# BlueAnon/BD-BNN

Measured on AMD Instinct MI355X. Metric: train_images_per_sec, higher is better.
Workload: dtype bf16; 1 GPU; model=resnet18_bdbnn, global_batch=2048, image=3x224x224, kurtosis=True, parallelism=dp1

## Files before the change

bdbnn_amd/csrc/api.h:

```cpp
#pragma once
#include <hip/hip_runtime.h>
#include <cstdint>

constexpr int BDBNN_MAX_TENSORS = 64;

struct TensorListArg {
  const float* ptr[BDBNN_MAX_TENSORS];
  int64_t numel[BDBNN_MAX_TENSORS];
  int n;
};

struct PtrList { float* ptr[BDBNN_MAX_TENSORS]; };

constexpr int64_t BDBNN_CHUNK_ELEMS = 32 * 1024;

constexpr int bdbnn_bn_sum_rows(int act_kind) {
  return act_kind == 3 ? 4 : 3;
}

extern "C" {

void bdbnn_sign_pack(const void* x, uint32_t* out, int64_t pixels, int C,
                     int CW, bool bf16, hipStream_t stream);
void bdbnn_binsign_decode(const void* x, void* y, int64_t n, bool in_bf16,
                          bool out_bf16, hipStream_t stream);
void bdbnn_ste_mask_mul(const void* g, const void* x, void* y, int64_t n,
                        bool g_bf16, bool x_bf16, int mode, float t, float k,
                        hipStream_t stream);
void bdbnn_weight_pack(const float* w, uint32_t* wp, float* alpha,
                       float* stab, int K, int C, int KH, int KW, int CW,
                       hipStream_t stream);
void bdbnn_sign_mask_pack(const void* x, uint32_t* sp, uint32_t* mp,
                          int64_t pixels, int C, int CW, bool bf16,
                          hipStream_t stream);
void bdbnn_decode_packed(const uint32_t* sp, void* y, int64_t pixels, int C,
                         int CW, bool out_bf16, hipStream_t stream);
void bdbnn_mask_mul_packed(const void* g, const uint32_t* mp, void* dx,
                           int64_t pixels, int C, int CW, bool g_bf16,
                           bool out_bf16, hipStream_t stream);
void bdbnn_weight_decode(const uint32_t* wp, const float* alpha, void* w,
                         int K, int C, int T, int CW, bool out_bf16,
                         hipStream_t stream);

void bdbnn_xnor_conv_fwd(
    const uint32_t* xp, const uint32_t* wp, const float* alpha,
    const float* stab, void* out, float* s1, float* s2, bool out_bf16,
    int N, int H, int W, int C, int K, int KH, int KW, int stride, int pad,
    int Ho, int Wo, hipStream_t stream);

void bdbnn_stem_pack_x4(const void* x, void* x4, int64_t npix, bool bf16,
                        hipStream_t stream);
void bdbnn_stem_pack_w4(const float* w, void* w4T, hipStream_t stream);
void bdbnn_stem_fwd(const void* x4, const void* w4T, void* out, int N, int H,
                    int W, hipStream_t stream);
int bdbnn_stem_wrw_nslab(int N, int H, int W);
void bdbnn_stem_wrw(const void* x4, const void* g, float* dwslab, int N,
                    int H, int W, hipStream_t stream);
void bdbnn_stem_fold_dw4(const float* slabs, float* dw, int nslab,
                         hipStream_t stream);

void bdbnn_kd_logit_fwd(const void* s, const void* t, float* stats,
                        float* out, int B, int C, bool bf16,
                        hipStream_t stream);
void bdbnn_kd_logit_bwd(const void* s, const void* t, const float* stats,
                        void* ds, float gscale, int B, int C, bool bf16,
                        hipStream_t stream);
void bdbnn_ce_fwd(const void* s, const int64_t* y, float* stats, float* out,
                  int B, int C, bool bf16, hipStream_t stream);
void bdbnn_ce_bwd(const void* s, const int64_t* y, const float* stats,
                  void* ds, float gscale, int B, int C, bool bf16,
                  hipStream_t stream);

void bdbnn_maxpool_fwd(const void* x, void* out, unsigned char* idx, int N,
                       int C, int H, int W, int Ho, int Wo, int ks,
                       int stride, int pad, bool bf16, hipStream_t stream);
void bdbnn_maxpool_bwd(const void* dy, const unsigned char* idx, void* dx,
                       int N, int C, int H, int W, int Ho, int Wo, int ks,
                       int stride, int pad, bool bf16, hipStream_t stream);

void bdbnn_prelu_fwd(const void* x, const float* a, void* y, int64_t n,
                     int C, bool bf16, hipStream_t stream);
void bdbnn_prelu_bwd(const void* x, const void* g, const float* a, void* dx,
                     float* da, int64_t n, int C, bool bf16,
                     hipStream_t stream);

void bdbnn_bn_stats(const void* x, float* s1, float* s2, int64_t n, int C,
                    bool bf16, hipStream_t stream);
void bdbnn_bn_finalize(const float* s1, const float* s2, float* mean,
                       float* invstd, float* running_mean,
                       float* running_var, int C, float n, float momentum,
                       float eps, int nslice, hipStream_t stream);
void bdbnn_bn_act_fwd(const void* x, const void* skip, const float* mean,
                      const float* invstd, const float* gamma,
                      const float* beta, const float* a, const float* b1,
                      const float* b2, void* out, void* zout, int64_t n,
                      int C, int act_kind, uint32_t* xpk, uint32_t* mpk,
                      bool bf16, hipStream_t stream);
void bdbnn_bn_act_bwd_reduce(const void* dy, const void* z, const void* x,
                             const float* mean, const float* invstd,
                             const float* a, float* sums32, float* sums,
                             int64_t n, int C, int act_kind, bool bf16,
                             hipStream_t stream);
void bdbnn_bn_fold_sums(const float* sums32, float* sums, int n,
                        hipStream_t stream);
void bdbnn_bn_act_bwd_apply(const void* dy, const void* z, const void* x,
                            const float* mean, const float* invstd,
                            const float* gamma, const float* a,
                            const float* sums, void* dx, void* dskip,
                            int64_t n, int C, int act_kind, float inv_n,
                            bool bf16, hipStream_t stream);
void bdbnn_bn_act_eval(const void* x, const void* skip, const float* rm,
                       const float* rv, const float* gamma,
                       const float* beta, const float* a, const float* b1,
                       const float* b2, void* out, int64_t n, int C,
                       int act_kind, float eps, bool bf16,
                       hipStream_t stream);

void bdbnn_bn_relu_maxpool_fwd(
    const void* x, const float* mean, const float* invstd,
    const float* gamma, const float* beta, void* out, unsigned char* idx,
    uint32_t* xpk, uint32_t* mpk, int N, int C, int H, int W, int Ho, int Wo,
    int ks, int stride, int pad, bool bf16, hipStream_t stream);
void bdbnn_bn_relu_maxpool_bwd_reduce(
    const void* dy, const unsigned char* idx, const void* x,
    const float* mean, const float* invstd, const float* gamma,
    const float* beta, float* sums32, float* sums, int N, int C, int H,
    int W, int Ho, int Wo, int ks, int stride, int pad, bool bf16,
    hipStream_t stream);
void bdbnn_bn_relu_maxpool_bwd_apply(
    const void* dy, const unsigned char* idx, const void* x,
    const float* mean, const float* invstd, const float* gamma,
// ... 61 lines not shown
```

bdbnn_amd/csrc/bind.cpp:

```cpp
#include <torch/extension.h>
#include <c10/hip/HIPStream.h>
#include <hip/hip_runtime.h>

#include <string>
#include <unordered_map>
#include <utility>
#include <vector>

#include "api.h"

namespace {

hipStream_t cur_stream() {
  return c10::hip::getCurrentHIPStream().stream();
}

bool is_bf16(const at::Tensor& t) { return t.scalar_type() == at::kBFloat16; }

void check_vec8(const at::Tensor& t, bool vec8_c, const char* name,
                const char* who) {
  TORCH_CHECK(t.is_cuda() && (t.scalar_type() == at::kBFloat16 ||
                              t.scalar_type() == at::kFloat),
              who, ": ", name, " must be a bf16 or fp32 CUDA tensor");
  if (vec8_c) {
    TORCH_CHECK(t.dim() == 4, who, ": ", name, " must be 4-D (N,C,H,W)");
    int64_t C = t.size(1);
    TORCH_CHECK(C >= 8 && C <= 1024 && (C & (C - 1)) == 0, who,
                ": C must be a power of two, 8 <= C <= 1024");
  }
}

struct Schedule {
  at::Tensor bt, bo;
  int n_blocks;
};

Schedule build_schedule_uncached(const std::vector<at::Tensor>& ts,
                                 int64_t chunk_elems, const at::Device& dev) {
  std::vector<int> bt;
  std::vector<int64_t> bo;
  for (size_t l = 0; l < ts.size(); ++l) {
    int64_t n = ts[l].numel();
    for (int64_t off = 0; off < n; off += chunk_elems) {
      bt.push_back((int)l);
      bo.push_back(off);
    }
  }
  Schedule s;
  s.n_blocks = (int)bt.size();
  s.bt = at::from_blob(bt.data(), {(int64_t)bt.size()},
                       at::TensorOptions().dtype(at::kInt))
             .to(dev, false);
  s.bo = at::from_blob(bo.data(), {(int64_t)bo.size()},
                       at::TensorOptions().dtype(at::kLong))
             .to(dev, false);
  return s;
}

Schedule build_schedule(const std::vector<at::Tensor>& ts,
                        int64_t chunk_elems, const at::Device& dev) {
  static std::unordered_map<std::string, Schedule> cache;
  std::string key;
  key.reserve(ts.size() * 9 + 16);
  key += std::to_string(chunk_elems);
  key += '/';
  key += std::to_string(dev.index());
  for (auto& t : ts) {
    key += ':';
    key += std::to_string(t.numel());
  }
  auto it = cache.find(key);
  if (it != cache.end()) return it->second;
  if (cache.size() > 256) cache.clear();
  auto s = build_schedule_uncached(ts, chunk_elems, dev);
  cache.emplace(std::move(key), s);
  return s;
}

TensorListArg make_meta(const std::vector<at::Tensor>& ts) {
  TORCH_CHECK((int)ts.size() <= BDBNN_MAX_TENSORS,
              "too many tensors for one fused call");
  TensorListArg a;
  a.n = (int)ts.size();
  for (size_t i = 0; i < ts.size(); ++i) {
    TORCH_CHECK((ts[i].is_contiguous() ||
                 ts[i].is_contiguous(at::MemoryFormat::ChannelsLast)) &&
// ... 159 lines not shown

at::Tensor ste_mask_mul(const at::Tensor& g, const at::Tensor& x, int mode,
                        double t, double k) {
  TORCH_CHECK(g.is_cuda() && x.is_cuda() && g.numel() == x.numel(),
              "ste_mask_mul: matching CUDA tensors");
  check_vec8(g, false, "g", "ste_mask_mul");
  check_vec8(x, false, "x", "ste_mask_mul");
  TORCH_CHECK(x.numel() % 8 == 0, "ste_mask_mul: numel % 8 == 0");
  auto fmt = x.dim() == 4 ? at::MemoryFormat::ChannelsLast
                          : at::MemoryFormat::Contiguous;
  auto xc = x.contiguous(fmt);
  auto gc = g.contiguous(fmt);
  auto out = at::empty_like(xc, xc.options(), fmt);
  bdbnn_ste_mask_mul(gc.data_ptr(), xc.data_ptr(), out.data_ptr(),
                     xc.numel(), is_bf16(gc), is_bf16(xc), mode, (float)t,
                     (float)k, cur_stream());
  return out;
}


std::vector<at::Tensor> sign_mask_pack_nhwc(const at::Tensor& x) {
  TORCH_CHECK(x.is_cuda() && x.dim() == 4, "sign_mask_pack: 4-D CUDA tensor");
  check_vec8(x, false, "x", "sign_mask_pack");
  TORCH_CHECK(x.is_contiguous(at::MemoryFormat::ChannelsLast),
              "sign_mask_pack: channels_last input required");
  int64_t N = x.size(0), C = x.size(1), H = x.size(2), W = x.size(3);
  int CW = (int)((C + 31) / 32);
  auto sp = at::empty({N, H, W, CW}, x.options().dtype(at::kInt));
  auto mp = at::empty({N, H, W, CW}, x.options().dtype(at::kInt));
  bdbnn_sign_mask_pack(x.data_ptr(), (uint32_t*)sp.data_ptr<int>(),
                       (uint32_t*)mp.data_ptr<int>(), N * H * W, (int)C, CW,
                       is_bf16(x), cur_stream());
  return {sp, mp};
}

at::Tensor decode_packed(const at::Tensor& sp, int64_t C, bool out_bf16) {
  TORCH_CHECK(sp.is_cuda() && sp.dim() == 4 && sp.scalar_type() == at::kInt,
              "decode_packed: int32 [N,H,W,CW]");
  int64_t N = sp.size(0), H = sp.size(1), W = sp.size(2);
  int CW = (int)sp.size(3);
  auto out = at::empty({N, C, H, W},
                       sp.options().dtype(out_bf16 ? at::kBFloat16
                                                   : at::kFloat),
                       at::MemoryFormat::ChannelsLast);
  bdbnn_decode_packed((const uint32_t*)sp.data_ptr<int>(), out.data_ptr(),
                      N * H * W, (int)C, CW, out_bf16, cur_stream());
  return out;
}

at::Tensor mask_mul_packed(const at::Tensor& g, const at::Tensor& mp,
                           int64_t C, bool out_bf16) {
  TORCH_CHECK(g.is_cuda() && mp.is_cuda(), "mask_mul_packed: CUDA tensors");
  check_vec8(g, false, "g", "mask_mul_packed");
  auto gc = g.contiguous(at::MemoryFormat::ChannelsLast);
  int64_t N = mp.size(0), H = mp.size(1), W = mp.size(2);
  int CW = (int)mp.size(3);
  TORCH_CHECK(gc.numel() == N * H * W * C, "mask_mul_packed: shape mismatch");
  auto out = at::empty({N, C, H, W},
                       g.options().dtype(out_bf16 ? at::kBFloat16
                                                  : at::kFloat),
                       at::MemoryFormat::ChannelsLast);
  bdbnn_mask_mul_packed(gc.data_ptr(), (const uint32_t*)mp.data_ptr<int>(),
                        out.data_ptr(), N * H * W, (int)C, CW, is_bf16(gc),
                        out_bf16, cur_stream());
  return out;
}

at::Tensor weight_decode(const at::Tensor& wp, const at::Tensor& alpha,
                         int64_t C, bool out_bf16) {
  TORCH_CHECK(wp.is_cuda() && wp.dim() == 4 && wp.scalar_type() == at::kInt,
              "weight_decode: int32 [K,KH,KW,CW]");
  int K = (int)wp.size(0), KH = (int)wp.size(1), KW = (int)wp.size(2);
  int CW = (int)wp.size(3);
  auto out = at::empty({K, C, KH, KW},
                       wp.options().dtype(out_bf16 ? at::kBFloat16
                                                   : at::kFloat));
  bdbnn_weight_decode((const uint32_t*)wp.data_ptr<int>(),
                      alpha.data_ptr<float>(), out.data_ptr(), K, (int)C,
                      KH * KW, CW, out_bf16, cur_stream());
  return out;
}


std::vector<at::Tensor> xnor_conv_fwd(
    const at::Tensor& xp, const at::Tensor& wp, const at::Tensor& alpha,
    const at::Tensor& stab, int64_t C, int64_t stride, int64_t pad,
    bool out_bf16, bool want_stats) {
  TORCH_CHECK(xp.is_cuda() && xp.dim() == 4 && xp.scalar_type() == at::kInt,
              "xnor_conv: packed activations int32 [N,H,W,CW]");
  TORCH_CHECK(wp.dim() == 4, "xnor_conv: packed weights [K,KH,KW,CW]");
  int N = (int)xp.size(0), H = (int)xp.size(1), W = (int)xp.size(2);
  int K = (int)wp.size(0), KH = (int)wp.size(1), KW = (int)wp.size(2);
  TORCH_CHECK(KH * KW * wp.size(3) <= 160,
              "xnor_conv: KH*KW*ceil(C/32) must be <= 160 "
              "(kernel address-table size; C <= 512 at 3x3)");
  int Ho = (int)((H + 2 * pad - KH) / stride + 1);
  int Wo = (int)((W + 2 * pad - KW) / stride + 1);
  auto out = at::empty({N, K, Ho, Wo},
                       xp.options().dtype(out_bf16 ? at::kBFloat16
                                                   : at::kFloat),
                       at::MemoryFormat::ChannelsLast);
  at::Tensor s1, s2;
  float *s1p = nullptr, *s2p = nullptr;
  if (want_stats) {
    auto fopt = xp.options().dtype(at::kFloat);
    s1 = at::empty({32, K}, fopt);
    s2 = at::empty({32, K}, fopt);
    s1p = s1.data_ptr<float>();
    s2p = s2.data_ptr<float>();
  }
  bdbnn_xnor_conv_fwd((const uint32_t*)xp.data_ptr<int>(),
                      (const uint32_t*)wp.data_ptr<int>(),
                      alpha.data_ptr<float>(), stab.data_ptr<float>(),
                      out.data_ptr(), s1p, s2p, out_bf16, N, H, W, (int)C,
                      K, KH, KW, (int)stride, (int)pad, Ho, Wo,
                      cur_stream());
  if (want_stats) return {out, s1, s2};
  return {out};
}



std::vector<at::Tensor> stem_conv_fwd(const at::Tensor& x,
                                      const at::Tensor& w) {
  TORCH_CHECK(x.is_cuda() && x.dim() == 4 && x.size(1) == 3,
              "stem: (N,3,H,W) input");
  TORCH_CHECK(w.dim() == 4 && w.size(0) == 64 && w.size(1) == 3 &&
                  w.size(2) == 7 && w.size(3) == 7,
              "stem: (64,3,7,7) weights");
  int N = (int)x.size(0), H = (int)x.size(2), W = (int)x.size(3);
  TORCH_CHECK(H % 2 == 0 && W % 2 == 0, "stem: even H,W");
  auto xc = x.contiguous(at::MemoryFormat::ChannelsLast);
  bool bf16 = is_bf16(xc);
  auto bopt = xc.options().dtype(at::kBFloat16);
  auto x4 = at::empty({N, H, W, 4}, bopt);
  bdbnn_stem_pack_x4(xc.data_ptr(), x4.data_ptr(), (int64_t)N * H * W,
                     bf16, cur_stream());
  auto wf = w.contiguous().to(at::kFloat);
  auto w4T = at::empty({64, 224}, bopt);
  bdbnn_stem_pack_w4(wf.data_ptr<float>(), w4T.data_ptr(), cur_stream());
  auto out = at::empty({N, 64, H / 2, W / 2}, bopt,
                       at::MemoryFormat::ChannelsLast);
  bdbnn_stem_fwd(x4.data_ptr(), w4T.data_ptr(), out.data_ptr(), N, H, W,
                 cur_stream());
  return {out, x4};
}

at::Tensor stem_conv_wrw(const at::Tensor& x4, const at::Tensor& gy) {
  TORCH_CHECK(x4.is_cuda() && x4.dim() == 4 && x4.size(3) == 4 &&
                  x4.scalar_type() == at::kBFloat16,
              "stem wrw: packed x4 (N,H,W,4) bf16");
  int N = (int)x4.size(0), H = (int)x4.size(1), W = (int)x4.size(2);
  auto gc = gy.to(at::kBFloat16).contiguous(at::MemoryFormat::ChannelsLast);
  TORCH_CHECK(gc.size(1) == 64 && gc.size(2) == H / 2 &&
                  gc.size(3) == W / 2, "stem wrw: grad shape");
  int nslab = bdbnn_stem_wrw_nslab(N, H, W);
  auto fopt = x4.options().dtype(at::kFloat);
  auto slabs = at::empty({nslab, 64, 224}, fopt);
  bdbnn_stem_wrw(x4.data_ptr(), gc.data_ptr(), slabs.data_ptr<float>(),
                 N, H, W, cur_stream());
  auto dw = at::empty({64, 3, 7, 7}, fopt);
  bdbnn_stem_fold_dw4(slabs.data_ptr<float>(), dw.data_ptr<float>(),
                      nslab, cur_stream());
  return dw;
}


std::vector<at::Tensor> kd_logit_fwd(const at::Tensor& s,
                                     const at::Tensor& t) {
  check_logits(s, "kd_logit_fwd");
  TORCH_CHECK(t.is_cuda() && s.sizes() == t.sizes(),
              "kd_logit_fwd: teacher logits must be a CUDA tensor of the "
              "student's shape");
  auto sc = s.contiguous();
  auto tc = t.to(s.scalar_type()).contiguous();
  int B = (int)s.size(0), C = (int)s.size(1);
  auto fopt = sc.options().dtype(at::kFloat);
  auto stats = at::empty({B, 4}, fopt);
  auto out = at::empty({}, fopt);
  bdbnn_kd_logit_fwd(sc.data_ptr(), tc.data_ptr(), stats.data_ptr<float>(),
                     out.data_ptr<float>(), B, C, is_bf16(sc),
                     cur_stream());
  return {out, stats, tc};
}

at::Tensor kd_logit_bwd(const at::Tensor& s, const at::Tensor& t,
                        const at::Tensor& stats, double gscale) {
  check_logits(s, "kd_logit_bwd");
  TORCH_CHECK(t.is_cuda() && t.scalar_type() == s.scalar_type() &&
                  t.sizes() == s.sizes() && t.is_contiguous(),
              "kd_logit_bwd: t must be contiguous, of s's dtype and shape");
  TORCH_CHECK(stats.is_cuda() && stats.scalar_type() == at::kFloat &&
                  stats.is_contiguous() && stats.numel() == 4 * s.size(0),
              "kd_logit_bwd: stats must be contiguous fp32 [B,4]");
  auto sc = s.contiguous();
  int B = (int)s.size(0), C = (int)s.size(1);
  auto ds = at::empty_like(sc);
  bdbnn_kd_logit_bwd(sc.data_ptr(), t.data_ptr(), stats.data_ptr<float>(),
                     ds.data_ptr(), (float)(gscale / B), B, C, is_bf16(sc),
                     cur_stream());
  return ds;
// ... 738 lines not shown
  auto st = stats.contiguous();
  auto gs = gscale.to(dev, at::kFloat).contiguous();
  bdbnn_kurtosis_bwd(&meta, &gp, sched.bt.data_ptr<int>(),
                     sched.bo.data_ptr<int64_t>(), sched.n_blocks,
                     st.data_ptr<float>(), tgt.data_ptr<float>(),
                     gs.data_ptr<float>(), cur_stream());
  return grads;
}


at::Tensor weight_kd_fwd(const std::vector<at::Tensor>& ws,
                         const std::vector<at::Tensor>& wt) {
  auto meta = make_meta(ws);
  auto sched = build_schedule(ws, BDBNN_CHUNK_ELEMS, ws[0].device());
  auto s_ptr = make_ptrs(ws, meta, ws);
  auto t_ptr = make_ptrs(wt, meta, ws);
  auto out = at::zeros({}, ws[0].options().dtype(at::kDouble));
  bdbnn_weight_kd_fwd(&meta, &s_ptr, &t_ptr, sched.bt.data_ptr<int>(),
                      sched.bo.data_ptr<int64_t>(), sched.n_blocks,
                      out.data_ptr<double>(), cur_stream());
  return out.to(at::kFloat);
}

std::vector<at::Tensor> weight_kd_bwd(const std::vector<at::Tensor>& wt,
                                      const at::Tensor& gscale) {
  auto meta = make_meta(wt);
  auto sched = build_schedule(wt, BDBNN_CHUNK_ELEMS, wt[0].device());
  auto t_ptr = make_ptrs(wt, meta, wt);
  std::vector<at::Tensor> grads;
  for (auto& t : wt)
    grads.push_back(at::empty_like(t, t.options(),
                                   at::MemoryFormat::Preserve));
  auto gp = make_ptrs(grads, meta, wt);
  auto gs = gscale.to(wt[0].device(), at::kFloat).contiguous();
  bdbnn_weight_kd_bwd(&meta, &t_ptr, &gp, sched.bt.data_ptr<int>(),
                      sched.bo.data_ptr<int64_t>(), sched.n_blocks,
                      gs.data_ptr<float>(), cur_stream());
  return grads;
}


void fused_sgd(const std::vector<at::Tensor>& p,
               const std::vector<at::Tensor>& g,
               const std::vector<at::Tensor>& buf, double lr, double momentum,
               double wd) {
  auto meta = make_meta(p);
  auto sched = build_schedule(p, BDBNN_CHUNK_ELEMS, p[0].device());
  auto pp = make_ptrs(p, meta, p);
  auto gg = make_ptrs(g, meta, p);
  auto bb = make_ptrs(buf, meta, p);
  bdbnn_fused_sgd(&meta, &pp, &gg, &bb, sched.bt.data_ptr<int>(),
                  sched.bo.data_ptr<int64_t>(), sched.n_blocks, (float)lr,
                  (float)momentum, (float)wd, cur_stream());
}

void fused_adam(const std::vector<at::Tensor>& p,
                const std::vector<at::Tensor>& g,
                const std::vector<at::Tensor>& m1,
                const std::vector<at::Tensor>& m2, double lr, double beta1,
                double beta2, double eps, double wd, double bc1, double bc2) {
  auto meta = make_meta(p);
  auto sched = build_schedule(p, BDBNN_CHUNK_ELEMS, p[0].device());
  auto pp = make_ptrs(p, meta, p);
  auto gg = make_ptrs(g, meta, p);
  auto mm1 = make_ptrs(m1, meta, p);
  auto mm2 = make_ptrs(m2, meta, p);
  bdbnn_fused_adam(&meta, &pp, &gg, &mm1, &mm2, sched.bt.data_ptr<int>(),
                   sched.bo.data_ptr<int64_t>(), sched.n_blocks, (float)lr,
                   (float)beta1, (float)beta2, (float)eps, (float)wd,
                   (float)bc1, (float)bc2, cur_stream());
}

PYBIND11_MODULE(TORCH_EXTENSION_NAME, m) {
  m.def("sign_pack_nhwc", &sign_pack_nhwc, "sign+bitpack NHWC activations");
  m.def("weight_pack", &weight_pack,
        "pack conv weights -> (bits, alpha, pad-correction table)");
  m.def("binsign_decode", &binsign_decode, "elementwise +-1 decode");
  m.def("ste_mask_mul", &ste_mask_mul, "quantizer backward mask multiply");
  m.def("sign_mask_pack_nhwc", &sign_mask_pack_nhwc,
        "pack sign + clip-STE mask bitplanes in one pass");
  m.def("decode_packed", &decode_packed, "packed signs -> +-1 NHWC tensor");
  m.def("mask_mul_packed", &mask_mul_packed, "dx = mask_bit ? g : 0");
  m.def("weight_decode", &weight_decode, "packed weights -> alpha*(+-1)");
  m.def("xnor_conv_fwd", &xnor_conv_fwd, "bit-packed XNOR+popcount conv");
  m.def("stem_conv_fwd", &stem_conv_fwd,
        "MFMA 7x7/2 stem conv fwd (returns out, packed x4)");
  m.def("stem_conv_wrw", &stem_conv_wrw, "MFMA stem conv weight grad");
  m.def("kd_logit_fwd", &kd_logit_fwd, "fused logit-KD fwd");
  m.def("kd_logit_bwd", &kd_logit_bwd, "fused logit-KD bwd");
  m.def("ce_fwd", &ce_fwd, "fused cross-entropy fwd");
  m.def("ce_bwd", &ce_bwd, "fused cross-entropy bwd");
  m.def("maxpool_fwd", &maxpool_fwd, "fused NHWC maxpool fwd (+u8 idx)");
  m.def("maxpool_bwd", &maxpool_bwd, "gather-based NHWC maxpool bwd");
  m.def("prelu_fwd", &prelu_fwd, "fused NHWC per-channel PReLU fwd");
  m.def("prelu_bwd", &prelu_bwd, "fused NHWC per-channel PReLU bwd");
  m.def("bn_act_fwd_train", &bn_act_fwd_train,
        "fused BN(+add)(+act) training forward -> [out, z, mean, invstd(, "
        "xpk, mpk)]; act_kind 3 (RPReLU) takes b1, b2 and stores u = z + b1 "
        "as z",
        py::arg("x"), py::arg("skip"), py::arg("gamma"), py::arg("beta"),
        py::arg("a"), py::arg("running_mean"), py::arg("running_var"),
        py::arg("momentum"), py::arg("eps"), py::arg("act_kind"),
        py::arg("pre_s1"), py::arg("pre_s2"), py::arg("want_pack"),
        py::arg("b1") = py::none(), py::arg("b2") = py::none());
  m.def("bn_act_bwd", &bn_act_bwd,
        "fused BN(+add)(+act) backward -> [dx, dskip, dgamma, dbeta, da]; "
        "act_kind 3 appends db1, db2");
  m.def("bn_act_eval", &bn_act_eval, "fused BN(+add)(+act) eval forward",
        py::arg("x"), py::arg("skip"), py::arg("gamma"), py::arg("beta"),
        py::arg("a"), py::arg("rm"), py::arg("rv"), py::arg("eps"),
        py::arg("act_kind"), py::arg("b1") = py::none(),
        py::arg("b2") = py::none());
  m.def("bn_relu_maxpool_fwd_train", &bn_relu_maxpool_fwd_train,
        "fused BN + ReLU + maxpool training forward -> [out, idx, mean, "
        "invstd(, xpk, mpk)]",
        py::arg("x"), py::arg("gamma"), py::arg("beta"),
        py::arg("running_mean"), py::arg("running_var"),
        py::arg("momentum"), py::arg("eps"), py::arg("ks"),
        py::arg("stride"), py::arg("pad"), py::arg("pre_s1") = py::none(),
        py::arg("pre_s2") = py::none(), py::arg("want_pack") = false);
  m.def("bn_relu_maxpool_bwd", &bn_relu_maxpool_bwd,
        "fused BN + ReLU + maxpool backward -> [dx, dgamma, dbeta]");
  m.def("conv_dgrad2", &conv_dgrad2,
        "MFMA bf16 dgrad v2: halo-staged 9-tap implicit GEMM with fused "
        "clip-STE mask (3x3/s1/p1); optional acc adds a same-shape "
        "skip-gradient tensor in the epilogue",
        py::arg("g"), py::arg("wd"), py::arg("mp"), py::arg("C"),
        py::arg("acc") = py::none());
  m.def("conv_dgrad2_x", &conv_dgrad2_x,
        "conv_dgrad2 with a value mask of the saved bf16 activation x in "
        "the epilogue: mode 1 = ReAct polynomial, 2 = EDE(t, k)",
        py::arg("g"), py::arg("wd"), py::arg("x"), py::arg("C"),
        py::arg("mode"), py::arg("t"), py::arg("k"),
        py::arg("acc") = py::none());
  m.def("dgrad_weight_decode", &dgrad_weight_decode,
        "packed bits -> mirrored transposed +-alpha bf16 [9][C][K]");
  m.def("dgrad2_supported",
        [](int64_t H, int64_t W, int64_t C, int64_t K) {
          return bdbnn_dgrad2_supported((int)H, (int)W, (int)C, (int)K) !=
                 0;
        },
        "shape support predicate for conv_dgrad2");
  m.def("conv_wgrad2", &conv_wgrad2,
        "MFMA bf16 wgrad v2: all-9-tap block GEMM from sign BITS "
        "(3x3/s1/p1) -> fp32 [9][C][K]");
  m.def("repack_cplane", &repack_cplane,
        "activation sign bits -> padded per-channel u64 row planes");
  m.def("wgrad_finish", &wgrad_finish,
        "dwT transpose to [K][C][3][3] + |w|<=1 STE mask, one pass");
  m.def("dgrad2_s2_supported",
        [](int64_t H, int64_t W, int64_t C, int64_t K, int64_t ks) {
          return dgrad2_s2_routed(H, W, C, K, ks);
        },
        "routing predicate of the stride-2 MFMA backward; H, W are the "
        "input (dx) size, ks in {3 (pad 1), 1 (pad 0)}; false also for "
        "the shapes the kernels run but lose on (3x3 with C >= 128 and "
        "K >= 256)",
        py::arg("H"), py::arg("W"), py::arg("C"), py::arg("K"),
        py::arg("ks"));
  m.def("conv_dgrad2_s2", &conv_dgrad2_s2,
        "MFMA bf16 dgrad of a 3x3/s2/p1 (wd [9][C][K]) or 1x1/s2/p0 (wd "
        "[1][C][K]) binary conv by pixel parity; mode 0 masks with the "
        "bitplane mp, modes 1/2 with the value mask of x; optional acc "
        "adds a same-shape skip-gradient tensor in the epilogue",
        py::arg("g"), py::arg("wd"), py::arg("H"), py::arg("W"),
        py::arg("C"), py::arg("mode"), py::arg("mp"), py::arg("x"),
        py::arg("t"), py::arg("k"), py::arg("acc") = py::none());
// ... 21 lines not shown
```

bdbnn_amd/csrc/xnor_conv.hip:

```cpp
#include "common.h"
#include <cstdlib>

#define TILE_K 64
#define CHUNK 8
#define W_PER_THREAD 2
#define MAX_WORDS 160

struct XnorConvParams {
  int N, H, W, C, K, KH, KW, stride, pad, Ho, Wo, CW;
  int WORDS;
  int T;
  int base;
};

template <typename TO, bool STATS, int TM>
__global__ __launch_bounds__(256) void xnor_conv_kernel(
    const uint32_t* __restrict__ xp, const uint32_t* __restrict__ wp,
    const float* __restrict__ alpha, const float* __restrict__ stab,
    TO* __restrict__ out, float* __restrict__ s1, float* __restrict__ s2,
    XnorConvParams p, int grid_m) {
  const int wg = bd_xcd_remap(blockIdx.x, gridDim.x);
  int m_blk = wg % grid_m;
  int k_blk = wg / grid_m;
  const int tid = threadIdx.x;
  const int64_t M = (int64_t)p.N * p.Ho * p.Wo;
  const int64_t m0 = (int64_t)m_blk * TM;
  const int k0_blk = k_blk * TILE_K;

  constexpr int APT = CHUNK * TM / 256;
  constexpr int RPT = TM / 16;
  __shared__ uint32_t a_lds[2][CHUNK][TM];
  __shared__ uint32_t w_lds[2][CHUNK][TILE_K];
  __shared__ int row_basecw[TM];
  __shared__ unsigned short row_inv[TM];
  __shared__ int off_tab[MAX_WORDS];
  __shared__ unsigned char tap_tab[MAX_WORDS];
  __shared__ float csum[2][TILE_K];

  for (int r = tid; r < TM; r += blockDim.x) {
    int64_t sp = m0 + r;
    if (sp >= M) { row_basecw[r] = 0; row_inv[r] = 0xffff; continue; }
    int n = int(sp / ((int64_t)p.Ho * p.Wo));
    int rem = int(sp % ((int64_t)p.Ho * p.Wo));
    int oy = rem / p.Wo, ox = rem % p.Wo;
    int iy0 = oy * p.stride - p.pad;
    int ix0 = ox * p.stride - p.pad;
    row_basecw[r] = ((n * p.H + iy0) * p.W + ix0) * p.CW;
    unsigned short inv = 0;
    for (int t = 0; t < p.T; ++t) {
      int kh = t / p.KW, kw = t % p.KW;
      int iy = iy0 + kh, ix = ix0 + kw;
      if (iy < 0 || iy >= p.H || ix < 0 || ix >= p.W) inv |= 1u << t;
    }
    row_inv[r] = inv;
  }
  for (int wdx = tid; wdx < p.WORDS; wdx += blockDim.x) {
    int t = wdx / p.CW, cw = wdx - t * p.CW;
    int kh = t / p.KW, kw = t - kh * p.KW;
    off_tab[wdx] = (kh * p.W + kw) * p.CW + cw;
    tap_tab[wdx] = (unsigned char)t;
  }
  if constexpr (STATS)
    for (int c = tid; c < TILE_K; c += blockDim.x) {
      csum[0][c] = 0.f; csum[1][c] = 0.f;
    }
  __syncthreads();

  const int r0 = (tid / 16) * RPT;
  const int kq = (tid % 16) * 4;
  int acc[RPT][4] = {};

  int a_c[APT], a_r[APT];
#pragma unroll
  for (int it = 0; it < APT; ++it) {
    int j = tid + it * 256;
    a_c[it] = j / TM;
    a_r[it] = j % TM;
  }
  int w_c[W_PER_THREAD], w_k[W_PER_THREAD];
#pragma unroll
  for (int it = 0; it < W_PER_THREAD; ++it) {
    int j = tid + it * 256;
    w_c[it] = j / TILE_K;
    w_k[it] = j % TILE_K;
  }

  const int n_chunks = (p.WORDS + CHUNK - 1) / CHUNK;
  uint32_t av[APT], wv[W_PER_THREAD];

#define STAGE_LOAD(w0)                                                    \
  {                                                                       \
    _Pragma("unroll")                                                     \
    for (int it = 0; it < APT; ++it) {                                    \
      int widx = (w0) + a_c[it];                                          \
      int r = a_r[it];                                                    \
      uint32_t v = 0;                                                     \
      if (widx < p.WORDS && !((row_inv[r] >> tap_tab[widx]) & 1))         \
        v = xp[(int64_t)row_basecw[r] + off_tab[widx]];                   \
      av[it] = v;                                                         \
    }                                                                     \
    _Pragma("unroll")                                                     \
    for (int it = 0; it < W_PER_THREAD; ++it) {                           \
      int widx = (w0) + w_c[it];                                          \
      int kg = k0_blk + w_k[it];                                          \
      uint32_t v = 0;                                                     \
      if (widx < p.WORDS && kg < p.K)                                     \
        v = wp[(int64_t)kg * p.WORDS + widx];                             \
      wv[it] = v;                                                         \
    }                                                                     \
  }

#define STAGE_WRITE(buf)                                                  \
  {                                                                       \
    _Pragma("unroll")                                                     \
    for (int it = 0; it < APT; ++it)                                      \
      a_lds[buf][a_c[it]][a_r[it]] = av[it];                              \
    _Pragma("unroll")                                                     \
    for (int it = 0; it < W_PER_THREAD; ++it)                             \
      w_lds[buf][w_c[it]][w_k[it]] = wv[it];                              \
  }

  STAGE_LOAD(0);
  STAGE_WRITE(0);
  __syncthreads();

  for (int ch = 0; ch < n_chunks; ++ch) {
    const int buf = ch & 1;
    const bool more = ch + 1 < n_chunks;
    if (more) STAGE_LOAD((ch + 1) * CHUNK);
#pragma unroll
    for (int c = 0; c < CHUNK; ++c) {
// ... 137 lines not shown
```

setup.py:

```python

import os

from setuptools import setup

os.environ.setdefault("PYTORCH_ROCM_ARCH", "gfx950")

from torch.utils.cpp_extension import BuildExtension, CUDAExtension

ROOT = os.path.dirname(os.path.abspath(__file__))
CSRC = os.path.join(ROOT, "bdbnn_amd", "csrc")

sources = [os.path.join(CSRC, f) for f in (
    "bind.cpp",
    "pack.hip",
    "prelu.hip",
    "bn_act.hip",
    "bn_pool.hip",
    "pool.hip",
    "loss.hip",
    "conv_bwd.hip",
    "conv_bwd_s2.hip",
    "stem_conv.hip",
    "xnor_conv.hip",
    "kurtosis.hip",
    "kd.hip",
    "optim.hip",
)]

setup(
    name="bdbnn_amd_native",
    ext_modules=[
        CUDAExtension(
            name="bdbnn_amd._native",
            sources=sources,
            extra_compile_args={
                "cxx": ["-O3", "-std=c++17"],
                "nvcc": ["-O3", "-std=c++17"],
            },
        )
    ],
    cmdclass={"build_ext": BuildExtension.with_options(no_python_abi_suffix=False)},
)
```

Before: 25150 images/s.

## Add i8 MFMA binary conv forward kernel routed for 3x3 shapes

Adds a new forward kernel for binary 3x3 convolutions (stride 1 or 2, pad 1). It expands bit-packed signs into ±1 int8 in LDS, using halo tiles with swizzled slots, and accumulates with 32x32x32 i8 MFMA instructions instead of XNOR+popcount on the vector ALUs. The bind layer sends calls to it automatically when no BN statistics are requested and the channel counts are multiples of 64; an env var can turn this off, and the old kernel's invalid-tap mask is widened to 32 bits. The trade is an 8x expansion of the operand bytes written to LDS, plus a path that only runs when the stats epilogue is not needed.

```diff
diff --git a/bdbnn_amd/csrc/api.h b/bdbnn_amd/csrc/api.h
--- a/bdbnn_amd/csrc/api.h
+++ b/bdbnn_amd/csrc/api.h
@@ -47,6 +47,15 @@
     const float* stab, void* out, float* s1, float* s2, bool out_bf16,
     int N, int H, int W, int C, int K, int KH, int KW, int stride, int pad,
     int Ho, int Wo, hipStream_t stream);
+
+int bdbnn_xnor_mfma_supported(int C, int K, int KH, int KW, int stride,
+                              int pad);
+int bdbnn_xnor_mfma_routed(int C, int K, int KH, int KW, int stride,
+                           int pad);
+int bdbnn_xnor_conv_mfma_fwd(
+    const uint32_t* xp, const uint32_t* wp, const float* alpha, void* out,
+    bool out_bf16, int N, int H, int W, int C, int K, int KH, int KW,
+    int stride, int pad, int Ho, int Wo, hipStream_t stream);
 
 void bdbnn_stem_pack_x4(const void* x, void* x4, int64_t npix, bool bf16,
                         hipStream_t stream);
diff --git a/bdbnn_amd/csrc/bind.cpp b/bdbnn_amd/csrc/bind.cpp
--- a/bdbnn_amd/csrc/bind.cpp
+++ b/bdbnn_amd/csrc/bind.cpp
@@ -2,6 +2,7 @@
 #include <c10/hip/HIPStream.h>
 #include <hip/hip_runtime.h>
 
+#include <atomic>
 #include <string>
 #include <unordered_map>
 #include <utility>
@@ -327,10 +328,14 @@
 }
 
 
-std::vector<at::Tensor> xnor_conv_fwd(
+enum XnorRoute { kAuto, kMfma, kValu };
+
+static std::atomic<int64_t> g_xnor_route_calls[2];
+
+std::vector<at::Tensor> xnor_conv_route(
     const at::Tensor& xp, const at::Tensor& wp, const at::Tensor& alpha,
     const at::Tensor& stab, int64_t C, int64_t stride, int64_t pad,
-    bool out_bf16, bool want_stats) {
+    bool out_bf16, bool want_stats, XnorRoute route) {
   TORCH_CHECK(xp.is_cuda() && xp.dim() == 4 && xp.scalar_type() == at::kInt,
               "xnor_conv: packed activations int32 [N,H,W,CW]");
   TORCH_CHECK(wp.dim() == 4, "xnor_conv: packed weights [K,KH,KW,CW]");
@@ -339,6 +344,8 @@
   TORCH_CHECK(KH * KW * wp.size(3) <= 160,
               "xnor_conv: KH*KW*ceil(C/32) must be <= 160 "
               "(kernel address-table size; C <= 512 at 3x3)");
+  TORCH_CHECK(KH * KW <= 32,
+              "xnor_conv: at most 32 taps (invalid-tap bitmask width)");
   int Ho = (int)((H + 2 * pad - KH) / stride + 1);
   int Wo = (int)((W + 2 * pad - KW) / stride + 1);
   auto out = at::empty({N, K, Ho, Wo},
@@ -354,14 +361,71 @@
     s1p = s1.data_ptr<float>();
     s2p = s2.data_ptr<float>();
   }
+  bool mfma = route == kMfma;
+  if (route == kAuto)
+    mfma = !want_stats && bdbnn_xnor_mfma_routed((int)C, K, KH, KW,
+                                                 (int)stride, (int)pad);
+  if (mfma) {
+    TORCH_CHECK(!want_stats, "xnor_conv_mfma: no BN statistics epilogue");
+    TORCH_CHECK(wp.size(3) * 32 == C && xp.size(3) == wp.size(3),
+                "xnor_conv_mfma: C must equal 32 * CW of both operands");
+    int rc = bdbnn_xnor_conv_mfma_fwd(
+        (const uint32_t*)xp.data_ptr<int>(),
+        (const uint32_t*)wp.data_ptr<int>(), alpha.data_ptr<float>(),
+        out.data_ptr(), out_bf16, N, H, W, (int)C, K, KH, KW, (int)stride,
+        (int)pad, Ho, Wo, cur_stream());
+    TORCH_CHECK(rc == 0, "xnor_conv_mfma: ",
+                rc == -1 ? "unsupported shape" : "tensor too large");
+    ++g_xnor_route_calls[0];
+    return {out};
+  }
   bdbnn_xnor_conv_fwd((const uint32_t*)xp.data_ptr<int>(),
                       (const uint32_t*)wp.data_ptr<int>(),
                       alpha.data_ptr<float>(), stab.data_ptr<float>(),
                       out.data_ptr(), s1p, s2p, out_bf16, N, H, W, (int)C,
                       K, KH, KW, (int)stride, (int)pad, Ho, Wo,
                       cur_stream());
+  ++g_xnor_route_calls[1];
   if (want_stats) return {out, s1, s2};
   return {out};
+}
+
+std::vector<at::Tensor> xnor_conv_fwd(
+    const at::Tensor& xp, const at::Tensor& wp, const at::Tensor& alpha,
+    const at::Tensor& stab, int64_t C, int64_t stride, int64_t pad,
+    bool out_bf16, bool want_stats) {
+  return xnor_conv_route(xp, wp, alpha, stab, C, stride, pad, out_bf16,
+                         want_stats, kAuto);
+}
+
+at::Tensor xnor_conv_mfma_fwd(const at::Tensor& xp, const at::Tensor& wp,
+                              const at::Tensor& alpha, int64_t C,
+                              int64_t stride, int64_t pad, bool out_bf16) {
+  TORCH_CHECK(wp.dim() == 4 &&
+                  bdbnn_xnor_mfma_supported((int)C, (int)wp.size(0),
+                                            (int)wp.size(1), (int)wp.size(2),
+                                            (int)stride, (int)pad),
+              "xnor_conv_mfma_fwd: shape not supported by the MFMA kernel");
+  return xnor_conv_route(xp, wp, alpha, alpha, C, stride, pad, out_bf16,
+                         false, kMfma)[0];
+}
+
+std::vector<at::Tensor> xnor_conv_valu_fwd(
+    const at::Tensor& xp, const at::Tensor& wp, const at::Tensor& alpha,
+    const at::Tensor& stab, int64_t C, int64_t stride, int64_t pad,
+    bool out_bf16, bool want_stats) {
+  return xnor_conv_route(xp, wp, alpha, stab, C, stride, pad, out_bf16,
+                         want_stats, kValu);
+}
+
+bool xnor_mfma_supported(int64_t C, int64_t K, int64_t KH, int64_t KW,
+                         int64_t stride, int64_t pad) {
+  return bdbnn_xnor_mfma_supported((int)C, (int)K, (int)KH, (int)KW,
+                                   (int)stride, (int)pad) != 0;
+}
+
+std::vector<int64_t> xnor_route_calls() {
+  return {g_xnor_route_calls[0].load(), g_xnor_route_calls[1].load()};
 }
 
 
@@ -1266,7 +1330,17 @@
   m.def("decode_packed", &decode_packed, "packed signs -> +-1 NHWC tensor");
   m.def("mask_mul_packed", &mask_mul_packed, "dx = mask_bit ? g : 0");
   m.def("weight_decode", &weight_decode, "packed weights -> alpha*(+-1)");
-  m.def("xnor_conv_fwd", &xnor_conv_fwd, "bit-packed XNOR+popcount conv");
+  m.def("xnor_conv_fwd", &xnor_conv_fwd,
+        "binary conv forward (i8 MFMA or XNOR+popcount, by the routing "
+        "table)");
+  m.def("xnor_mfma_supported", &xnor_mfma_supported,
+        "(C, K, KH, KW, stride, pad): can the i8 MFMA forward run it");
+  m.def("xnor_conv_mfma_fwd", &xnor_conv_mfma_fwd,
+        "binary conv forward, i8 MFMA kernel forced");
+  m.def("xnor_conv_valu_fwd", &xnor_conv_valu_fwd,
+        "binary conv forward, XNOR+popcount kernel forced");
+  m.def("xnor_route_calls", &xnor_route_calls,
+        "(MFMA, VALU) forward conv calls since load");
   m.def("stem_conv_fwd", &stem_conv_fwd,
         "MFMA 7x7/2 stem conv fwd (returns out, packed x4)");
   m.def("stem_conv_wrw", &stem_conv_wrw, "MFMA stem conv weight grad");
diff --git a/bdbnn_amd/csrc/xnor_conv.hip b/bdbnn_amd/csrc/xnor_conv.hip
--- a/bdbnn_amd/csrc/xnor_conv.hip
+++ b/bdbnn_amd/csrc/xnor_conv.hip
@@ -32,21 +32,21 @@
   __shared__ uint32_t a_lds[2][CHUNK][TM];
   __shared__ uint32_t w_lds[2][CHUNK][TILE_K];
   __shared__ int row_basecw[TM];
-  __shared__ unsigned short row_inv[TM];
+  __shared__ uint32_t row_inv[TM];
   __shared__ int off_tab[MAX_WORDS];
   __shared__ unsigned char tap_tab[MAX_WORDS];
   __shared__ float csum[2][TILE_K];
 
   for (int r = tid; r < TM; r += blockDim.x) {
     int64_t sp = m0 + r;
-    if (sp >= M) { row_basecw[r] = 0; row_inv[r] = 0xffff; continue; }
+    if (sp >= M) { row_basecw[r] = 0; row_inv[r] = 0xffffffffu; continue; }
     int n = int(sp / ((int64_t)p.Ho * p.Wo));
     int rem = int(sp % ((int64_t)p.Ho * p.Wo));
     int oy = rem / p.Wo, ox = rem % p.Wo;
     int iy0 = oy * p.stride - p.pad;
     int ix0 = ox * p.stride - p.pad;
     row_basecw[r] = ((n * p.H + iy0) * p.W + ix0) * p.CW;
-    unsigned short inv = 0;
+    uint32_t inv = 0;
     for (int t = 0; t < p.T; ++t) {
       int kh = t / p.KW, kw = t % p.KW;
       int iy = iy0 + kh, ix = ix0 + kw;
diff --git a/bdbnn_amd/csrc/xnor_conv_mfma.hip b/bdbnn_amd/csrc/xnor_conv_mfma.hip
--- /dev/null
+++ b/bdbnn_amd/csrc/xnor_conv_mfma.hip
@@ -0,0 +1,297 @@
+#include "conv_bwd_common.h"
+#include <cstdlib>
+
+typedef __attribute__((ext_vector_type(4))) int i32x4;
+typedef __attribute__((ext_vector_type(16))) int i32x16;
+
+#define XM_BM 256
+#define XM_BN 64
+#define XM_BK 64
+
+struct XnorMfmaParams {
+  int N, H, W, Ho, Wo, K, CW;
+  int segs;
+  int bands_per_image;
+  int total_slots;
+};
+
+__device__ __forceinline__ uint32_t xm_spread4(uint32_t nib) {
+  return (nib * 0x00204081u) & 0x01010101u;
+}
+
+template <bool INV>
+__device__ __forceinline__ uint4 xm_expand16(uint32_t bits) {
+  uint32_t v[4];
+#pragma unroll
+  for (int i = 0; i < 4; ++i) {
+    uint32_t m = xm_spread4((bits >> (4 * i)) & 0xfu) * 0xfeu;
+    v[i] = INV ? (m ^ 0x01010101u) : ~m;
+  }
+  return uint4{v[0], v[1], v[2], v[3]};
+}
+
+__device__ __forceinline__ int xm_slot(int row, int q) {
+  return row * XM_BK + ((q ^ ((row >> 1) & 3)) << 4);
+}
+
+template <typename TO, int S, int WP, int RB, int GB>
+__global__ __launch_bounds__(512, 2) void xnor_conv_mfma_kernel(
+    const uint32_t* __restrict__ xp, const uint32_t* __restrict__ wp,
+    const float* __restrict__ alpha, TO* __restrict__ out, XnorMfmaParams p,
+    int grid_m) {
+  constexpr int HR = (RB - 1) * S + 3;
+  constexpr int WH = (WP - 1) * S + 3;
+  constexpr int NHE = GB * HR * WH;
+  constexpr int AW = NHE * 2;
+  constexpr int APT = (AW + 511) / 512;
+  constexpr int WROWS = 9 * XM_BN;
+  constexpr int WW = WROWS * 2;
+  constexpr int WPT = (WW + 511) / 512;
+
+  const int wg = bd_xcd_remap(blockIdx.x, gridDim.x);
+  const int tile = wg % grid_m;
+  const int k0 = (wg / grid_m) * XM_BN;
+  const int tid = threadIdx.x;
+
+  __shared__ __align__(16) unsigned char halo[NHE * XM_BK];
+  __shared__ __align__(16) unsigned char wlds[WROWS * XM_BK];
+  __shared__ int he_base[NHE];
+  __shared__ int tab_he[XM_BM];
+  __shared__ int tab_out[XM_BM];
+
+  const int slot0 = tile * GB;
+  for (int he = tid; he < NHE; he += 512) {
+    int band = he / (HR * WH);
+    int rem = he - band * (HR * WH);
+    int hr = rem / WH, hx = rem - hr * WH;
+    int slot = slot0 + band;
+    int base = -1;
+    if (slot < p.total_slots) {
+      int n = slot / (p.bands_per_image * p.segs);
+      int r2 = slot - n * (p.bands_per_image * p.segs);
+      int bi = r2 / p.segs, seg = r2 - bi * p.segs;
+      int iy = bi * RB * S - 1 + hr;
+      int ix = seg * WP * S - 1 + hx;
+      if (iy >= 0 && iy < p.H && ix >= 0 && ix < p.W)
+        base = (n * p.H + iy) * p.W + ix;
+    }
+    he_base[he] = base;
+  }
+  for (int m = tid; m < XM_BM; m += 512) {
+    int band = m / (RB * WP);
+    int rem = m - band * (RB * WP);
+    int rloc = rem / WP, x = rem - rloc * WP;
+    int slot = slot0 + band;
+    tab_he[m] = band * (HR * WH) + rloc * S * WH + x * S;
+    int o = -1;
+    if (slot < p.total_slots) {
+      int n = slot / (p.bands_per_image * p.segs);
+      int r2 = slot - n * (p.bands_per_image * p.segs);
+      int bi = r2 / p.segs, seg = r2 - bi * p.segs;
+      int oy = bi * RB + rloc, ox = seg * WP + x;
+      if (oy < p.Ho && ox < p.Wo) o = (n * p.Ho + oy) * p.Wo + ox;
+    }
+    tab_out[m] = o;
+  }
+  __syncthreads();
+
+  const int wid = tid >> 6, lane = tid & 63;
+  const int wm0 = (wid >> 1) * 64;
+  const int wc = (wid & 1) * 32;
+  const int lrow = lane & 31, lh = lane >> 5;
+  const int he0 = tab_he[wm0 + lrow];
+  const int he1 = tab_he[wm0 + 32 + lrow];
+
+  i32x16 acc0, acc1;
+#pragma unroll
+  for (int i = 0; i < 16; ++i) { acc0[i] = 0; acc1[i] = 0; }
+
+  uint32_t areg[APT], wreg[WPT];
+  bool aval[APT];
+
+#define XM_LOAD(ci)                                                       \
+  {                                                                       \
+    _Pragma("unroll")                                                     \
+    for (int it = 0; it < APT; ++it) {                                    \
+      int i = tid + it * 512;                                             \
+      uint32_t v = 0;                                                     \
+      bool ok = false;                                                    \
+      if (i < AW) {                                                       \
+        int base = he_base[i >> 1];                                       \
+        if (base >= 0) {                                                  \
+          v = xp[(int64_t)base * p.CW + (ci) * 2 + (i & 1)];              \
+          ok = true;                                                      \
+        }                                                                 \
+      }                                                                   \
+      areg[it] = v;                                                       \
+      aval[it] = ok;                                                      \
+    }                                                                     \
+    _Pragma("unroll")                                                     \
+    for (int it = 0; it < WPT; ++it) {                                    \
+      int i = tid + it * 512;                                             \
+      uint32_t v = 0;                                                     \
+      if (i < WW) {                                                       \
+        int row = i >> 1;                                \
+        int t = row >> 6, kb = row & 63;                                  \
+        v = wp[((int64_t)(k0 + kb) * 9 + t) * p.CW + (ci) * 2 + (i & 1)]; \
+      }                                                                   \
+      wreg[it] = v;                                                       \
+    }                                                                     \
+  }
+
+#define XM_WRITE()                                                        \
+  {                                                                       \
+    _Pragma("unroll")                                                     \
+    for (int it = 0; it < APT; ++it) {                                    \
+      int i = tid + it * 512;                                             \
+      if (i < AW) {                                                       \
+        int he = i >> 1, q = (i & 1) * 2;                                 \
+        uint4 lo{0, 0, 0, 0}, hi{0, 0, 0, 0};                             \
+        if (aval[it]) {                                                   \
+          lo = xm_expand16<false>(areg[it] & 0xffffu);                    \
+          hi = xm_expand16<false>(areg[it] >> 16);                        \
+        }                                                                 \
+        *(uint4*)&halo[xm_slot(he, q)] = lo;                              \
+        *(uint4*)&halo[xm_slot(he, q + 1)] = hi;                          \
+      }                                                                   \
+    }                                                                     \
+    _Pragma("unroll")                                                     \
+    for (int it = 0; it < WPT; ++it) {                                    \
+      int i = tid + it * 512;                                             \
+      if (i < WW) {                                                       \
+        int row = i >> 1, q = (i & 1) * 2;                                \
+        *(uint4*)&wlds[xm_slot(row, q)] =                                 \
+            xm_expand16<true>(wreg[it] & 0xffffu);                        \
+        *(uint4*)&wlds[xm_slot(row, q + 1)] =                             \
+            xm_expand16<true>(wreg[it] >> 16);                            \
+      }                                                                   \
+    }                                                                     \
+  }
+
+  const int n_chunks = p.CW / 2;
+  XM_LOAD(0);
+  for (int ci = 0; ci < n_chunks; ++ci) {
+    const bool more = ci + 1 < n_chunks;
+    XM_WRITE();
+    __syncthreads();
+    if (more) XM_LOAD(ci + 1);
+#pragma unroll
+    for (int t = 0; t < 9; ++t) {
+      const int dy = t / 3, dx = t - dy * 3;
+      const int hA = he0 + dy * WH + dx;
+      const int hB = he1 + dy * WH + dx;
+      const int wr = t * XM_BN + wc + lrow;
+#pragma unroll
+      for (int kk = 0; kk < 2; ++kk) {
+        const int q = kk * 2 + lh;
+        i32x4 a = *(const i32x4*)&wlds[xm_slot(wr, q)];
+        i32x4 b0 = *(const i32x4*)&halo[xm_slot(hA, q)];
+        i32x4 b1 = *(const i32x4*)&halo[xm_slot(hB, q)];
+        acc0 = __builtin_amdgcn_mfma_i32_32x32x32_i8(a, b0, acc0, 0, 0, 0);
+        acc1 = __builtin_amdgcn_mfma_i32_32x32x32_i8(a, b1, acc1, 0, 0, 0);
+      }
+    }
+    if (more) __syncthreads();
+  }
+#undef XM_LOAD
+#undef XM_WRITE
+
+  float al[16];
+#pragma unroll
+  for (int g = 0; g < 4; ++g)
+    *(float4*)&al[4 * g] =
+        *(const float4*)&alpha[k0 + wc + mfma32_cd_row(4 * g, lh)];
+#pragma unroll
+  for (int half = 0; half < 2; ++half) {
+    const i32x16& acc = half ? acc1 : acc0;
+    const int pix = tab_out[wm0 + half * 32 + lrow];
+    if (pix < 0) continue;
+    TO* dst = out + (int64_t)pix * p.K + k0 + wc;
+#pragma unroll
+    for (int g = 0; g < 4; ++g) {
+      const int ch = mfma32_cd_row(4 * g, lh);
+      if constexpr (sizeof(TO) == 2) {
+        uint16_t vals[4];
+#pragma unroll
+        for (int j = 0; j < 4; ++j)
+          vals[j] = f32_to_bf16(al[4 * g + j] * float(acc[4 * g + j]));
+        *(uint2*)&dst[ch] = *(uint2*)vals;
+      } else {
+        float vals[4];
+#pragma unroll
+        for (int j = 0; j < 4; ++j)
+          vals[j] = al[4 * g + j] * float(acc[4 * g + j]);
+        *(float4*)&dst[ch] = *(float4*)vals;
+      }
+    }
+  }
+}
+
+
+template <class F>
+static int xnor_mfma_class(int Wo, F f) {
+  if (Wo <= 8) return f(BwdClass<8, 8, 4>{});
+  if (Wo <= 16) return f(BwdClass<16, 16, 1>{});
+  if (Wo <= 32) return f(BwdClass<32, 8, 1>{});
+  return f(BwdClass<64, 4, 1>{});
+}
+
+template <class F>
+static int xnor_mfma_route_class(int C, int K, int KH, int KW, int stride,
+                                 int pad, F f) {
+  if (KH != 3 || KW != 3 || pad != 1) return -1;
+  if (C <= 0 || C % XM_BK || K <= 0 || K % XM_BN) return -1;
+  if (stride == 1) return f(true);
+  if (stride == 2) return f(true);
+  return -1;
+}
+
+extern "C" int bdbnn_xnor_mfma_supported(int C, int K, int KH, int KW,
+                                         int stride, int pad) {
+  return xnor_mfma_route_class(C, K, KH, KW, stride, pad,
+                               [](bool) { return 0; }) == 0;
+}
+
+extern "C" int bdbnn_xnor_mfma_routed(int C, int K, int KH, int KW,
+                                      int stride, int pad) {
+  static const bool knob = [] {
+    const char* e = getenv("BDBNN_XNOR_MFMA");
+    return e ? atoi(e) != 0 : true;
+  }();
+  if (!knob) return 0;
+  return xnor_mfma_route_class(C, K, KH, KW, stride, pad,
+                               [](bool on) { return on ? 1 : 0; }) == 1;
+}
+
+extern "C" int bdbnn_xnor_conv_mfma_fwd(
+    const uint32_t* xp, const uint32_t* wp, const float* alpha, void* out,
+    bool out_bf16, int N, int H, int W, int C, int K, int KH, int KW,
+    int stride, int pad, int Ho, int Wo, hipStream_t stream) {
+  if (!bdbnn_xnor_mfma_supported(C, K, KH, KW, stride, pad)) return -1;
+  if ((int64_t)N * H * W > INT32_MAX || (int64_t)N * Ho * Wo > INT32_MAX)
+    return -2;
+  return xnor_mfma_class(Wo, [&](auto cls) {
+    using G = decltype(cls);
+    XnorMfmaParams p;
+    p.N = N; p.H = H; p.W = W; p.Ho = Ho; p.Wo = Wo; p.K = K;
+    p.CW = C / 32;
+    p.segs = (Wo + G::WP - 1) / G::WP;
+    p.bands_per_image = (Ho + G::RB - 1) / G::RB;
+    int64_t slots = (int64_t)N * p.bands_per_image * p.segs;
+    int64_t blocks = (slots + G::GB - 1) / G::GB * (K / XM_BN);
+    if (slots > INT32_MAX || blocks > INT32_MAX) return -2;
+    p.total_slots = (int)slots;
+    int grid_m = (int)((slots + G::GB - 1) / G::GB);
+    dim3 grid((unsigned)blocks);
+    with_dtype(out_bf16, [&](auto t) {
+      using TO = decltype(t);
+      if (stride == 1)
+        xnor_conv_mfma_kernel<TO, 1, G::WP, G::RB, G::GB>
+            <<<grid, 512, 0, stream>>>(xp, wp, alpha, (TO*)out, p, grid_m);
+      else
+        xnor_conv_mfma_kernel<TO, 2, G::WP, G::RB, G::GB>
+            <<<grid, 512, 0, stream>>>(xp, wp, alpha, (TO*)out, p, grid_m);
+    });
+    return 0;
+  });
+}
diff --git a/setup.py b/setup.py
--- a/setup.py
+++ b/setup.py
@@ -22,6 +22,7 @@
     "conv_bwd_s2.hip",
     "stem_conv.hip",
     "xnor_conv.hip",
+    "xnor_conv_mfma.hip",
     "kurtosis.hip",
     "kd.hip",
     "optim.hip",
```

Result: faster. 27340 images/s (median of 6 runs) (+8.7%).
